# wangxiaohit/GNNPN-SC

Measured on AMD Instinct MI355X. Metric: service-composition problems/sec (ML+2PN inference), higher is better.
Workload: dtype f32-split3xf16 (f32 operands and results; recurrent W_hh.h products: fp32 operands split exactly into 3 x f16, six f16-matrix-core products per term, f32 accumulate; everything else f32 arithmetic)

## Files before the change

gnnpn-sc_amd/csrc/coop_common.h:

```cpp
#pragma once
#include "common.h"
#include "lstm_shared.h"

typedef float f32x4 __attribute__((ext_vector_type(4)));
typedef unsigned long long u64;

__device__ __forceinline__ void granule_store(u64* p, unsigned tag, float v) {
    __hip_atomic_store(p, ((u64)tag << 32) | __float_as_uint(v), __ATOMIC_RELAXED,
                       __HIP_MEMORY_SCOPE_AGENT);
}

typedef unsigned u32x4 __attribute__((ext_vector_type(4)));
#define GNNPN_LD2(dst, voff, sbase, off) "global_load_dwordx4 " dst ", " voff ", " sbase " offset:" off " sc1\n\t"
__device__ __forceinline__ const u64* uniform_ptr(const u64* p) {
    const unsigned long long v = (unsigned long long)p;
    const unsigned lo = __builtin_amdgcn_readfirstlane((unsigned)v), hi = __builtin_amdgcn_readfirstlane((unsigned)(v >> 32));
    return reinterpret_cast<const u64*>(((unsigned long long)hi << 32) | lo);
}
__device__ __forceinline__ void granule_reload2_x8_masked(u32x4 (&v)[8], const u64* base, unsigned voff, unsigned long long lanes) {
    const u64* q = base + 512;
    unsigned long long saved;
    asm volatile("s_and_saveexec_b64 %8, %12\n\t"
                 GNNPN_LD2("%0", "%9", "%10", "0") GNNPN_LD2("%1", "%9", "%10", "1024") GNNPN_LD2("%2", "%9", "%10", "2048")
                 GNNPN_LD2("%3", "%9", "%10", "3072") GNNPN_LD2("%4", "%9", "%11", "0") GNNPN_LD2("%5", "%9", "%11", "1024")
                 GNNPN_LD2("%6", "%9", "%11", "2048") GNNPN_LD2("%7", "%9", "%11", "3072")
                 "s_waitcnt vmcnt(0)\n\t"
                 "s_mov_b64 exec, %8"
                 : "+v"(v[0]), "+v"(v[1]), "+v"(v[2]), "+v"(v[3]), "+v"(v[4]), "+v"(v[5]), "+v"(v[6]), "+v"(v[7]), "=&s"(saved)
                 : "v"(voff), "s"(base), "s"(q), "s"(lanes)
                 : "memory", "scc");
}
__device__ __forceinline__ void granule_load2_x8_x4(u32x4 (&v)[8], u32x4 (&w)[4], const u64* base, const u64* pbase, unsigned voff) {
    const u64* q = base + 512;
    asm volatile(GNNPN_LD2("%0", "%12", "%13", "0") GNNPN_LD2("%1", "%12", "%13", "1024") GNNPN_LD2("%2", "%12", "%13", "2048")
                 GNNPN_LD2("%3", "%12", "%13", "3072") GNNPN_LD2("%4", "%12", "%14", "0") GNNPN_LD2("%5", "%12", "%14", "1024")
                 GNNPN_LD2("%6", "%12", "%14", "2048") GNNPN_LD2("%7", "%12", "%14", "3072")
                 GNNPN_LD2("%8", "%12", "%15", "0") GNNPN_LD2("%9", "%12", "%15", "1024") GNNPN_LD2("%10", "%12", "%15", "2048")
                 GNNPN_LD2("%11", "%12", "%15", "3072")
                 "s_waitcnt vmcnt(0)"
                 : "=&v"(v[0]), "=&v"(v[1]), "=&v"(v[2]), "=&v"(v[3]), "=&v"(v[4]), "=&v"(v[5]), "=&v"(v[6]), "=&v"(v[7]),
                   "=&v"(w[0]), "=&v"(w[1]), "=&v"(w[2]), "=&v"(w[3])
                 : "v"(voff), "s"(base), "s"(q), "s"(pbase)
                 : "memory");
}

__device__ __forceinline__ void granule_load2_x8_x4_lat(u32x4 (&v)[8], u32x4 (&w)[4], u64& lat, const u64* base, const u64* pbase,
                                                        const u64* lbase, unsigned voff) {
    const u64* q = base + 512;
    asm volatile(GNNPN_LD2("%0", "%13", "%15", "0") GNNPN_LD2("%1", "%13", "%15", "1024") GNNPN_LD2("%2", "%13", "%15", "2048")
                 GNNPN_LD2("%3", "%13", "%15", "3072") GNNPN_LD2("%4", "%13", "%16", "0") GNNPN_LD2("%5", "%13", "%16", "1024")
                 GNNPN_LD2("%6", "%13", "%16", "2048") GNNPN_LD2("%7", "%13", "%16", "3072")
                 GNNPN_LD2("%8", "%13", "%17", "0") GNNPN_LD2("%9", "%13", "%17", "1024") GNNPN_LD2("%10", "%13", "%17", "2048")
                 GNNPN_LD2("%11", "%13", "%17", "3072")
                 "global_load_dwordx2 %12, %14, %18 sc1\n\t"
                 "s_waitcnt vmcnt(0)"
                 : "=&v"(v[0]), "=&v"(v[1]), "=&v"(v[2]), "=&v"(v[3]), "=&v"(v[4]), "=&v"(v[5]), "=&v"(v[6]), "=&v"(v[7]),
                   "=&v"(w[0]), "=&v"(w[1]), "=&v"(w[2]), "=&v"(w[3]), "=&v"(lat)
                 : "v"(voff), "v"(voff >> 1), "s"(base), "s"(q), "s"(pbase), "s"(lbase)
                 : "memory");
}

constexpr int COOP_STAFFING_WORD = 8 * 256 + 8;
__device__ __forceinline__ void coop_raise(unsigned* err, unsigned* sticky, unsigned code, unsigned* seats = nullptr) {
    atomicOr(err, code);
    if (sticky) atomicOr(sticky, code);
    if (seats && atomicCAS(err + 4, 1u, 2u) == 1u) atomicSub(seats + COOP_STAFFING_WORD, 1u);
}

constexpr int COOP_STATUS_BYTES = 16384;
constexpr unsigned COOP_LDS_UNITS = 640;
constexpr int COOP_XCD_STRIDE = 32;
constexpr int COOP_XCDCNT_OFFSET = 12288;
constexpr int COOP_ARRIVE_OFFSET = 13312;
constexpr int COOP_PLACED_OFFSET = 14336;
constexpr int COOP_CLAIM_OFFSET = 2048;
constexpr int COOP_TAKEN_OFFSET = 10240;
constexpr int COOP_OVERREAD_BYTES = 4096;
constexpr int COOP_OVERSUB = 3;
constexpr unsigned COOP_SURPLUS_WAIT_TICKS = 1600;
constexpr unsigned COOP_RESERVE_WAIT_TICKS = 200000;

__device__ __forceinline__ unsigned xcc_id() {
// ... 249 lines not shown
        __builtin_amdgcn_sched_barrier(0);
        if (ch == 64 / CH / 2 - 1) mid();
    }
}

typedef _Float16 f16x8 __attribute__((ext_vector_type(8)));
constexpr int LDH16 = 264;
constexpr int SPLIT_TILE = 16 * LDH16;
constexpr float SPLIT_SCALE = 2048.0f, SPLIT_INV = 1.0f / 2048.0f;
constexpr float SPLIT_H_SCALE = 32768.0f, SPLIT_H_INV = 1.0f / 32768.0f;

__device__ __forceinline__ void split3(float xs, _Float16& p0, _Float16& p1, _Float16& p2) {
    p0 = (_Float16)xs;
    const float r1 = __fmul_rn(__fsub_rn(xs, (float)p0), SPLIT_SCALE);
    p1 = (_Float16)r1;
    p2 = (_Float16)__fmul_rn(__fsub_rn(r1, (float)p1), SPLIT_SCALE);
}
__device__ __forceinline__ unsigned short f16_bits(_Float16 v) { return __builtin_bit_cast(unsigned short, v); }

__device__ __forceinline__ unsigned split_tag16(unsigned tag) { return 0x8000u | (tag & 0x7fffu); }
__device__ __forceinline__ u64 split_granule(unsigned tag, float h) {
    _Float16 p0, p1, p2;
    split3(__fmul_rn(h, SPLIT_H_SCALE), p0, p1, p2);
    const unsigned d0 = (unsigned)f16_bits(p0) | (split_tag16(tag) << 16);
    const unsigned d1 = (unsigned)f16_bits(p1) | ((unsigned)f16_bits(p2) << 16);
    return ((u64)d1 << 32) | d0;
}
__device__ __forceinline__ void split_granule_store(u64* p, unsigned tag, float h, bool same_xcd) {
    const u64 g = split_granule(tag, h);
    if (same_xcd) granule_store_l2_bits(p, g);
    else __hip_atomic_store(p, g, __ATOMIC_RELAXED, __HIP_MEMORY_SCOPE_AGENT);
}
__device__ __forceinline__ bool split_pair_tagged(u32x4 v, unsigned tag) {
    const unsigned t = split_tag16(tag);
    return __builtin_amdgcn_perm(v.z, v.x, 0x07060302u) == (t | (t << 16));
}
__device__ __forceinline__ void split_pair_to_lds(_Float16* at, u32x4 v) {
    unsigned* d = reinterpret_cast<unsigned*>(at);
    d[0] = __builtin_amdgcn_perm(v.z, v.x, 0x05040100u);
    d[SPLIT_TILE / 2] = __builtin_amdgcn_perm(v.w, v.y, 0x05040100u);
    d[SPLIT_TILE] = __builtin_amdgcn_perm(v.w, v.y, 0x07060302u);
}
__device__ __forceinline__ void split_store(_Float16* at, float h) {
    _Float16 p0, p1, p2;
    split3(__fmul_rn(h, SPLIT_H_SCALE), p0, p1, p2);
    at[0] = p0;
    at[SPLIT_TILE] = p1;
    at[2 * SPLIT_TILE] = p2;
}

constexpr int SPLIT_WT_DWORDS = 4 * 8 * 64 * 4;
template <int HD>
__device__ __forceinline__ float split_weights(const float* __restrict__ Wp, int gate, int u, int kq, f16x8 (&w0)[8],
                                               f16x8 (&w1)[8], unsigned* wt) {
    float m = 0.0f;
#pragma unroll
    for (int kk = 0; kk < 8; ++kk)
#pragma unroll
        for (int j = 0; j < 8; ++j)
            m = fmaxf(m, fabsf(Wp[((size_t)((8 * kk + 2 * kq + (j >> 2)) * 4 + gate) * HD + u) * 4 + (j & 3)]));
    m = fmaxf(m, __shfl_xor(m, 16, 64));
    m = fmaxf(m, __shfl_xor(m, 32, 64));
    int e = 0;
    if (m > 0.0f && m < 3.0e38f) (void)frexpf(m, &e);
    int s = m > 0.0f ? 15 - e : 0;
    s = s > 96 ? 96 : (s < -96 ? -96 : s);
    const float up = ldexpf(1.0f, s);
#pragma unroll
    for (int kk = 0; kk < 8; ++kk) {
        unsigned bytes[2] = {0u, 0u};
#pragma unroll
        for (int j = 0; j < 8; ++j) {
            const float w = Wp[((size_t)((8 * kk + 2 * kq + (j >> 2)) * 4 + gate) * HD + u) * 4 + (j & 3)];
            _Float16 p0, p1, p2;
            split3(__fmul_rn(w, up), p0, p1, p2);
            w0[kk][j] = p0;
            w1[kk][j] = p1;
            bytes[j >> 2] |= (unsigned)(f16_bits(p2) >> 8) << (8 * (j & 3));
        }
        wt[4 * 64 * kk] = bytes[0];
        wt[4 * 64 * kk + 1] = bytes[1];
    }
    return ldexpf(1.0f, -(15 + s));
}
constexpr int SPLIT_PACK_U4_PER_MEMBER = 2 * 2 * 8 * 256 + 8 * 256 + 2 * 256 / 4;
constexpr int SPLIT_PACK_MEMBERS = 8;
__device__ __forceinline__ void load_split_weights(const uint4* __restrict__ pk, int tid, f16x8 (&w0)[2][8], f16x8 (&w1)[2][8],
                                                   unsigned* wt_lane, float (&inv)[2]) {
#pragma unroll
    for (int tl = 0; tl < 2; ++tl)
#pragma unroll
        for (int kk = 0; kk < 8; ++kk) {
            w0[tl][kk] = __builtin_bit_cast(f16x8, pk[((tl * 2 + 0) * 8 + kk) * 256 + tid]);
            w1[tl][kk] = __builtin_bit_cast(f16x8, pk[((tl * 2 + 1) * 8 + kk) * 256 + tid]);
        }
#pragma unroll
    for (int kk = 0; kk < 8; ++kk) *reinterpret_cast<uint4*>(wt_lane + 4 * 64 * kk) = pk[8192 + kk * 256 + tid];
    const float* fi = reinterpret_cast<const float*>(pk + 10240);
    inv[0] = fi[tid];
    inv[1] = fi[256 + tid];
}

__device__ __forceinline__ f16x8 split_expand(unsigned lo, unsigned hi) {
    const u32x4 r = {__builtin_amdgcn_perm(0u, lo, 0x010c000cu), __builtin_amdgcn_perm(0u, lo, 0x030c020cu),
                     __builtin_amdgcn_perm(0u, hi, 0x010c000cu), __builtin_amdgcn_perm(0u, hi, 0x030c020cu)};
    return __builtin_bit_cast(f16x8, r);
}
template <typename Mid = NoHook>
__device__ __forceinline__ void split_chain(const _Float16* base, const f16x8 (&w0)[2][8], const f16x8 (&w1)[2][8],
                                            const unsigned* wt, const float (&inv)[2], f32x4 (&acc)[2], Mid mid = Mid()) {
    constexpr int NT = 2;
    f32x4 a0[NT], a0b[NT], a1[NT], a2[NT];
#pragma unroll
    for (int n = 0; n < NT; ++n) a0[n] = a0b[n] = a1[n] = a2[n] = f32x4{0.f, 0.f, 0.f, 0.f};
    f16x8 h0[2];
    h0[0] = *reinterpret_cast<const f16x8*>(base);
    f16x8 h1 = *reinterpret_cast<const f16x8*>(base + SPLIT_TILE);
    f16x8 h2 = *reinterpret_cast<const f16x8*>(base + 2 * SPLIT_TILE);
    u32x4 t = *reinterpret_cast<const u32x4*>(wt);
#define GNNPN_FENCE __builtin_amdgcn_sched_barrier(0)
#pragma unroll
    for (int kk = 0; kk < 8; ++kk) {
        const int nx = 32 * (kk + 1), cur = kk & 1;
        u32x4 e0, e1;
        if (kk < 7) h0[cur ^ 1] = *reinterpret_cast<const f16x8*>(base + nx);
        GNNPN_FENCE;
        a2[0] = __builtin_amdgcn_mfma_f32_16x16x32_f16(h1, w1[0][kk], a2[0], 0, 0, 0);
        e0.x = __builtin_amdgcn_perm(0u, t.x, 0x010c000cu);
        e0.y = __builtin_amdgcn_perm(0u, t.x, 0x030c020cu);
        GNNPN_FENCE;
        a2[1] = __builtin_amdgcn_mfma_f32_16x16x32_f16(h1, w1[1][kk], a2[1], 0, 0, 0);
        e0.z = __builtin_amdgcn_perm(0u, t.y, 0x010c000cu);
        e0.w = __builtin_amdgcn_perm(0u, t.y, 0x030c020cu);
        GNNPN_FENCE;
        a1[0] = __builtin_amdgcn_mfma_f32_16x16x32_f16(h1, w0[0][kk], a1[0], 0, 0, 0);
        e1.x = __builtin_amdgcn_perm(0u, t.z, 0x010c000cu);
        e1.y = __builtin_amdgcn_perm(0u, t.z, 0x030c020cu);
        GNNPN_FENCE;
        a1[1] = __builtin_amdgcn_mfma_f32_16x16x32_f16(h1, w0[1][kk], a1[1], 0, 0, 0);
        e1.z = __builtin_amdgcn_perm(0u, t.w, 0x010c000cu);
        e1.w = __builtin_amdgcn_perm(0u, t.w, 0x030c020cu);
        GNNPN_FENCE;
        if (kk < 7) {
            h1 = *reinterpret_cast<const f16x8*>(base + SPLIT_TILE + nx);
            t = *reinterpret_cast<const u32x4*>(wt + 4 * 64 * (kk + 1));
        }
        a2[0] = __builtin_amdgcn_mfma_f32_16x16x32_f16(h0[cur], __builtin_bit_cast(f16x8, e0), a2[0], 0, 0, 0);
        GNNPN_FENCE;
        a2[1] = __builtin_amdgcn_mfma_f32_16x16x32_f16(h0[cur], __builtin_bit_cast(f16x8, e1), a2[1], 0, 0, 0);
        GNNPN_FENCE;
        if (kk < 4) a0[0] = __builtin_amdgcn_mfma_f32_16x16x32_f16(h0[cur], w0[0][kk], a0[0], 0, 0, 0);
        else a0b[0] = __builtin_amdgcn_mfma_f32_16x16x32_f16(h0[cur], w0[0][kk], a0b[0], 0, 0, 0);
        GNNPN_FENCE;
        if (kk < 4) a0[1] = __builtin_amdgcn_mfma_f32_16x16x32_f16(h0[cur], w0[1][kk], a0[1], 0, 0, 0);
        else a0b[1] = __builtin_amdgcn_mfma_f32_16x16x32_f16(h0[cur], w0[1][kk], a0b[1], 0, 0, 0);
        GNNPN_FENCE;
        a2[0] = __builtin_amdgcn_mfma_f32_16x16x32_f16(h2, w0[0][kk], a2[0], 0, 0, 0);
        GNNPN_FENCE;
        a2[1] = __builtin_amdgcn_mfma_f32_16x16x32_f16(h2, w0[1][kk], a2[1], 0, 0, 0);
        GNNPN_FENCE;
        if (kk < 7) h2 = *reinterpret_cast<const f16x8*>(base + 2 * SPLIT_TILE + nx);
        a1[0] = __builtin_amdgcn_mfma_f32_16x16x32_f16(h0[cur], w1[0][kk], a1[0], 0, 0, 0);
        GNNPN_FENCE;
        a1[1] = __builtin_amdgcn_mfma_f32_16x16x32_f16(h0[cur], w1[1][kk], a1[1], 0, 0, 0);
        GNNPN_FENCE;
        if (kk == 3) mid();
    }
#undef GNNPN_FENCE
#pragma unroll
    for (int n = 0; n < NT; ++n)
#pragma unroll
        for (int r = 0; r < 4; ++r)
            acc[n][r] = __fmul_rn(fmaf(fmaf(a2[n][r], SPLIT_INV, a1[n][r]), SPLIT_INV, __fadd_rn(a0[n][r], a0b[n][r])), inv[n]);
}

__device__ __forceinline__ void cell_update_split(const f32x2 (&g0)[2], const f32x2 (&g1)[2], bool lo_half, f32x2& cst, f32x2& h) {
    f32x2 a0[2], a1[2];
#pragma unroll
    for (int q = 0; q < 2; ++q) {
        a0[q] = cell_act2(g0[q], false);
        a1[q] = cell_act2(g1[q], lo_half);
    }
    const f32x2 s0 = lo_half ? a0[1] : a0[0], s1 = lo_half ? a1[1] : a1[0];
    const f32x2 t0 = {swap8(s0.x), swap8(s0.y)}, t1 = {swap8(s1.x), swap8(s1.y)};
    const f32x2 ig = lo_half ? a0[0] : t0, gg = lo_half ? a1[0] : t1;
    const f32x2 fg = lo_half ? t0 : a0[1], og = lo_half ? t1 : a1[1];
    cst = fg * cst + ig * gg;
    h = og * cell_act2(cst, true);
}
```

gnnpn-sc_amd/csrc/lstm_coop.hip:

```cpp
#include "common.h"
#include "recurrent.h"
#include "lstm_shared.h"
#include "coop_common.h"
#include "decode_shared.h"

namespace {
constexpr int H = COOP_H;
constexpr int G = COOP_G;
constexpr int ROWS = COOP_ROWS;
constexpr int UNITS = H / G;
constexpr unsigned SPIN_LIMIT = 400000;
constexpr int GROUP_GRANULES = 2 * ROWS * H + 2 * 4 * G;
constexpr int ENC_LOOP_PAD_NOPS = 13;
}

template <int PREC>
__device__ __forceinline__ bool sweep_quarter(const u64* buf, unsigned tag, float* hs, int wave, int lane, bool keep,
                                              bool nowait = false) {
    const u64* src = uniform_ptr(buf + wave * 4 * H);
    const unsigned voff = 16u * lane;
    u32x4 v[8];
#pragma unroll
    for (int j = 0; j < 8; ++j) asm volatile("" : "=v"(v[j]));
    bool bad = true;
    unsigned spins = 0;
    int nap = 1;
    for (;;) {
        granule_reload2_x8_masked(v, src, voff, __ballot(bad));
        bad = false;
#pragma unroll
        for (int j = 0; j < 8; ++j) {
            if constexpr (PREC == 2) bad |= !split_pair_tagged(v[j], tag);
            else bad |= (v[j].y != tag) | (v[j].w != tag);
        }
        if (!__any(bad) || nowait) break;
        if (++spins > SPIN_LIMIT) return false;
        for (int z = 0; z < nap; ++z) __builtin_amdgcn_s_sleep(2);
        if (nap < 16) nap <<= 1;
    }
    if (keep) {
#pragma unroll
        for (int j = 0; j < 8; ++j) {
            const int i = 2 * (j * 64 + lane);
            if constexpr (PREC == 0) {
                float* d = &hs[ht_index(wave * 4 + (i >> 8), i & 255)];
                d[0] = __uint_as_float(v[j].x);
                d[64] = __uint_as_float(v[j].z);
            } else {
                _Float16* h16 = reinterpret_cast<_Float16*>(hs) + (wave * 4 + (i >> 8)) * LDH16 + (i & 255);
                if constexpr (PREC == 2) {
                    split_pair_to_lds(h16, v[j]);
                } else {
                    h16[0] = (_Float16)__uint_as_float(v[j].x);
                    h16[1] = (_Float16)__uint_as_float(v[j].z);
                }
            }
        }
    }
    return true;
}


template <int PREC, bool PRE, bool DIAG>
__global__ __launch_bounds__(256, 2) void lstm_encode_coop_kernel(LstmNets nets, u64* __restrict__ xchg,
                                                                  unsigned* __restrict__ err, unsigned* __restrict__ sticky,
                                                                  int32_t B, int32_t L, int n_nets, int groups_per_net,
                                                                  int gpx, int ablate_arg, unsigned* __restrict__ seats,
                                                                  unsigned* __restrict__ diag) {
    const int ablate = DIAG ? (ablate_arg & ~0x1000) : (ablate_arg & 128);
    constexpr bool F16 = PREC != 0, SPLIT = PREC == 2;
    constexpr int HS_FLOATS = PREC == 2 ? 3 * SPLIT_TILE / 2 : ROWS * LDH16;
    __shared__ __attribute__((aligned(16))) float hs[HS_FLOATS];
    __shared__ __attribute__((aligned(16))) float hst[ROWS][UNITS];
    __shared__ int abort_flag;

    const int lane = threadIdx.x & 63, wave = threadIdx.x >> 6;
    const int kq = lane >> 4, c = lane & 15;
    __shared__ int place[2];
    int group, member;
    u64 p_entry = 0, p_placed = 0, p_weights = 0;
    if constexpr (DIAG) p_entry = phase_stamp();
    if (!coop_place<G>(err, gpx, place, group, member, seats, (ablate_arg & 0x1000) != 0, sticky)) return;
    if constexpr (DIAG) p_placed = phase_stamp();
    const int net = group / groups_per_net, gi = group % groups_per_net;
    if (net >= n_nets) return;
    if (threadIdx.x == 0) abort_flag = 0;
    __syncthreads();
    const bool same_xcd = !(ablate & 128);
    if (threadIdx.x == 0 && same_xcd) atomicAdd(err + COOP_PLACED_OFFSET / 4 + COOP_XCD_STRIDE * xcc_id(), 1u);

    const float* __restrict__ pre = PRE ? nets.pregates[net] : nullptr;
    const float* __restrict__ xin = nets.inputs[net];
    const float* __restrict__ Wp = nets.whh[net];
    float* __restrict__ enc = nets.enc_out[net];
    u64* xg = xchg + (size_t)group * GROUP_GRANULES;

    const int unit = member * UNITS + wave * 8 + (c & 7);
    int wrow[2];
    wrow[0] = (0 + (c >> 3)) * H + unit;
    wrow[1] = (2 + (c >> 3)) * H + unit;
    float wB[F16 ? 1 : 2][F16 ? 1 : 64], bh[2], wX[2][2] = {{0.f, 0.f}, {0.f, 0.f}}, bx[2] = {0.f, 0.f};
    f16x8 wB16[F16 ? 2 : 1][8];
    f16x8 wL16[SPLIT ? 2 : 1][8];
    float winv[2] = {1.0f, 1.0f};
    __shared__ __attribute__((aligned(16))) unsigned wts[SPLIT ? SPLIT_WT_DWORDS : 4];
    unsigned* wt_lane = wts + (SPLIT ? (wave * 8 * 64 + lane) * 4 : 0);
    const uint4* __restrict__ Wsplit = SPLIT ? static_cast<const uint4*>(nets.whh_split[net]) : nullptr;
    if constexpr (SPLIT) {
        if (Wsplit) load_split_weights(Wsplit + (size_t)member * SPLIT_PACK_U4_PER_MEMBER, threadIdx.x, wB16, wL16, wt_lane, winv);
    }
#pragma unroll
    for (int tl = 0; tl < 2; ++tl) {
        const int gate = wrow[tl] / H, u = wrow[tl] % H;
        bh[tl] = nets.bhh[net][wrow[tl]];
        if constexpr (SPLIT) {
            if (!Wsplit) winv[tl] = split_weights<H>(Wp, gate, u, kq, wB16[tl], wL16[tl], wt_lane + 2 * tl);
        } else if constexpr (F16) {
#pragma unroll
            for (int kk = 0; kk < 8; ++kk)
#pragma unroll
                for (int j = 0; j < 8; ++j)
                    wB16[tl][kk][j] = (_Float16)Wp[((size_t)((8 * kk + 2 * kq + (j >> 2)) * 4 + gate) * H + u) * 4 + (j & 3)];
        }
        if constexpr (!PRE) {
            wX[tl][0] = nets.w_in[net][wrow[tl] * 8 + kq];
            wX[tl][1] = nets.w_in[net][wrow[tl] * 8 + 4 + kq];
            bx[tl] = nets.b_in[net][wrow[tl]];
        }
        if constexpr (!F16) {
#pragma unroll
            for (int kk = 0; kk < 64; ++kk)
                wB[tl][kk] = Wp[((size_t)(kk * 4 + gate) * H + u) * 4 + kq];
        }
    }

    if constexpr (DIAG) {
        asm volatile("" ::"v"(winv[0]), "v"(winv[1]), "v"(bh[0]), "v"(bh[1]));
        p_weights = phase_stamp();
    }
    const int n_tiles = (B + ROWS - 1) / ROWS;
    unsigned step = 0;
    unsigned tiles_done = 0;
    bool first_tile = true;
    for (int tile = gi; tile < n_tiles; tile += groups_per_net) {
        const int b0 = tile * ROWS;
        f32x2 cst = {0.f, 0.f};
        f32x2 hlast = {0.f, 0.f};
        float pg[2][4], pg_next[2][4] = {{0.f, 0.f, 0.f, 0.f}, {0.f, 0.f, 0.f, 0.f}};
        float ax[2] = {0.f, 0.f}, ax_next[2] = {0.f, 0.f};
        auto load_input = [&](int t, float (&pgv)[2][4], float (&axv)[2]) {
            if constexpr (PRE) {
#pragma unroll
                for (int r = 0; r < 4; ++r) {
                    const int b = b0 + kq * 4 + r;
#pragma unroll
                    for (int tl = 0; tl < 2; ++tl)
                        pgv[tl][r] = b < B ? pre[((int64_t)b * L + t) * (4 * H) + wrow[tl]] : 0.0f;
                }
            } else if (b0 + c < B) {
                const float* row = xin + ((int64_t)(b0 + c) * L + t) * 8;
                axv[0] = row[kq];
                axv[1] = row[4 + kq];
            }
        };
        load_input(0, pg_next, ax_next);
#ifndef GNNPN_ENC_PAD_NOPS
#define GNNPN_ENC_PAD_NOPS ENC_LOOP_PAD_NOPS
#endif
        if constexpr (SPLIT && !DIAG) asm volatile(".p2align 6\n\t.rept %0\n\ts_nop 0\n\t.endr" ::"n"(GNNPN_ENC_PAD_NOPS) : "memory");
        for (int t = 0; t < L; ++t, ++step) {
            const bool stamps = ablate & 32;
            u64 s0 = 0, s1 = 0, s2 = 0, s3 = 0, s4 = 0, s5 = 0;
            if (stamps) s0 = phase_stamp();
#pragma unroll
            for (int tl = 0; tl < 2; ++tl) {
                ax[tl] = ax_next[tl];
#pragma unroll
                for (int r = 0; r < 4; ++r) pg[tl][r] = pg_next[tl][r];
            }
            f32x4 px0 = {0.f, 0.f, 0.f, 0.f}, px1 = {0.f, 0.f, 0.f, 0.f};
            if constexpr (!PRE) {
                px0 = __builtin_amdgcn_mfma_f32_16x16x4f32(ax[0], wX[0][0], px0, 0, 0, 0);
                px1 = __builtin_amdgcn_mfma_f32_16x16x4f32(ax[0], wX[1][0], px1, 0, 0, 0);
                px0 = __builtin_amdgcn_mfma_f32_16x16x4f32(ax[1], wX[0][1], px0, 0, 0, 0);
                px1 = __builtin_amdgcn_mfma_f32_16x16x4f32(ax[1], wX[1][1], px1, 0, 0, 0);
            }
            bool ok = true;
            if (t == 0) {
                for (int i = threadIdx.x; i < HS_FLOATS; i += 256) hs[i] = 0.0f;
                if (!first_tile) ok = sweep_quarter<PREC>(xg + ((step - 1) & 1) * (ROWS * H), step, hs, wave, lane, false);
            } else if (!(ablate & 8)) {
                ok = sweep_quarter<PREC>(xg + ((step - 1) & 1) * (ROWS * H), step, hs, wave, lane, true, ablate & 4);
            }
            if (!ok) abort_flag = 1;
            if constexpr (DIAG) {
                if (!ok && lane == 0 && diag) {
                    const unsigned n = atomicAdd(diag, 1u);
                    if (n < 31) {
                        unsigned* rec = diag + 16 * (n + 1);
                        const unsigned* cnt = err + COOP_XCDCNT_OFFSET / 4;
                        const unsigned* arr = err + COOP_ARRIVE_OFFSET / 4;
                        unsigned c0 = 0, c1 = 0, a0 = 0, a1 = 0;
                        for (int x = 0; x < 4; ++x) {
                            c0 |= (cnt[COOP_XCD_STRIDE * x] & 0xffu) << (8 * x);
                            c1 |= (cnt[COOP_XCD_STRIDE * (4 + x)] & 0xffu) << (8 * x);
                            a0 |= (arr[COOP_XCD_STRIDE * x] & 0xffu) << (8 * x);
                            a1 |= (arr[COOP_XCD_STRIDE * (4 + x)] & 0xffu) << (8 * x);
                        }
                        rec[0] = group; rec[1] = member; rec[2] = tile; rec[3] = t; rec[4] = wave; rec[5] = step;
                        rec[6] = 0; rec[7] = 0xE0Cu; rec[8] = 0; rec[9] = c0; rec[10] = c1; rec[11] = a0; rec[12] = a1;
                        rec[13] = gpx; rec[14] = blockIdx.x; rec[15] = err[0];
                    }
                }
            }
            if (stamps) s1 = phase_stamp();
            __syncthreads();
            if (abort_flag) break;
            if (stamps) s2 = phase_stamp();
            f32x4 acc0 = {0.f, 0.f, 0.f, 0.f}, acc1 = {0.f, 0.f, 0.f, 0.f};
            u64 s2a = 0;
            if (stamps) s2a = phase_stamp();
            if constexpr (SPLIT) {
                if (t > 0) {
                    f32x4 acc[2] = {acc0, acc1};
                    split_chain(reinterpret_cast<const _Float16*>(hs) + c * LDH16 + 8 * kq, wB16, wL16, wt_lane, winv, acc);
                    acc0 = acc[0];
                    acc1 = acc[1];
                }
            } else if constexpr (F16) {
                if (t > 0) {
                    const _Float16* base = reinterpret_cast<const _Float16*>(hs) + c * LDH16 + 8 * kq;
                    f16x8 a16[8];
#pragma unroll
                    for (int kk = 0; kk < 8; ++kk) a16[kk] = *reinterpret_cast<const f16x8*>(base + 32 * kk);
#pragma unroll
                    for (int kk = 0; kk < 8; ++kk) {
                        acc0 = __builtin_amdgcn_mfma_f32_16x16x32_f16(a16[kk], wB16[0][kk], acc0, 0, 0, 0);
                        acc1 = __builtin_amdgcn_mfma_f32_16x16x32_f16(a16[kk], wB16[1][kk], acc1, 0, 0, 0);
                    }
                }
            } else {
                if (t > 0 && !(ablate & 1)) mfma_chain_pair<LDT, 16, true>(hs, c, kq, wB[0], wB[F16 ? 0 : 1], acc0, acc1);
            }
            if (t + 1 < L && !(ablate & 0x400)) load_input(t + 1, pg_next, ax_next);
            if (t > 0 && threadIdx.x < ROWS * 8 && !(ablate & 0x200)) {
                const int row = threadIdx.x >> 3, q = threadIdx.x & 7;
                if (b0 + row < B)
                    *reinterpret_cast<float4*>(enc + ((int64_t)(b0 + row) * L + (t - 1)) * H + member * UNITS + 4 * q) =
                        *reinterpret_cast<const float4*>(&hst[row][4 * q]);
            }

            if (stamps) {
                asm volatile("" ::"v"(acc0[0]), "v"(acc1[0]));
                s3 = phase_stamp();
            }
            if constexpr (!PRE) {
#pragma unroll
                for (int r = 0; r < 4; ++r) {
                    pg[0][r] = __fadd_rn(px0[r], bx[0]);
                    pg[1][r] = __fadd_rn(px1[r], bx[1]);
                }
            }
            __syncthreads();
            if (stamps) s4 = phase_stamp();

            u64* out_buf = xg + (step & 1) * (ROWS * H);
            {
                f32x2 g0[2], g1[2];
#pragma unroll
                for (int q = 0; q < 2; ++q) {
                    g0[q] = (f32x2{acc0[2 * q], acc0[2 * q + 1]} + pk_set(bh[0])) + f32x2{pg[0][2 * q], pg[0][2 * q + 1]};
                    g1[q] = (f32x2{acc1[2 * q], acc1[2 * q + 1]} + pk_set(bh[1])) + f32x2{pg[1][2 * q], pg[1][2 * q + 1]};
                }
                cell_update_split(g0, g1, c < 8, cst, hlast);
            }
            {
                const int r0 = kq * 4 + (c < 8 ? 0 : 2);
                u64* dst = out_buf + r0 * H + unit;
                if constexpr (SPLIT) {
                    split_granule_store(dst, step + 1, hlast.x, same_xcd);
                    split_granule_store(dst + H, step + 1, hlast.y, same_xcd);
                } else if (!(ablate & 16)) {
                    if (same_xcd) {
                        granule_store_l2(dst, step + 1, hlast.x);
                        granule_store_l2(dst + H, step + 1, hlast.y);
                    } else {
                        granule_store(dst, step + 1, hlast.x);
                        granule_store(dst + H, step + 1, hlast.y);
                    }
                }
                hst[r0][wave * 8 + (c & 7)] = hlast.x;
                hst[r0 + 1][wave * 8 + (c & 7)] = hlast.y;
            }
            if (stamps) {
                asm volatile("" ::"v"(hlast.y));
                s5 = phase_stamp();
                if (blockIdx.x == 0 && threadIdx.x == 0 && t > 0) {
                    u64* prof = reinterpret_cast<u64*>(err) + 4;
                    prof[0] += s1 - s0;
                    prof[1] += s2 - s1;
                    prof[2] += s3 - s2;
                    prof[6] += s2a - s2;
                    prof[3] += s4 - s3;
                    prof[4] += s5 - s4;
                    prof[5] += 1;
                    if (t == 1 && first_tile) {
                        prof[7] = p_placed - p_entry;
                        prof[8] = p_weights - p_placed;
                        prof[9] = s0 - p_weights;
                    }
                }
            }
        }
        if (abort_flag) break;
        __syncthreads();
        if (threadIdx.x < ROWS * 8) {
            const int row = threadIdx.x >> 3, q = threadIdx.x & 7;
            if (b0 + row < B)
                *reinterpret_cast<float4*>(enc + ((int64_t)(b0 + row) * L + (L - 1)) * H + member * UNITS + 4 * q) =
                    *reinterpret_cast<const float4*>(&hst[row][4 * q]);
        }
#pragma unroll
        for (int r = 0; r < 2; ++r) {
            const int b = b0 + kq * 4 + (c < 8 ? 0 : 2) + r;
            if (b < B) {
                nets.h_n[net][(int64_t)b * H + unit] = r ? hlast.y : hlast.x;
                nets.c_n[net][(int64_t)b * H + unit] = r ? cst.y : cst.x;
            }
        }
        first_tile = false;
        ++tiles_done;
    }
    if (threadIdx.x == 0) {
        if (abort_flag) coop_raise(err, sticky, 1u, seats);
        coop_note_finished(sticky, GNNPN_STATUS_ENC_FINISHED, tiles_done);
    }
}


__global__ __launch_bounds__(256) void lstm_pack_split_kernel(const float* __restrict__ Wp, uint4* __restrict__ out) {
    __shared__ __attribute__((aligned(16))) unsigned wts[SPLIT_WT_DWORDS];
    const int tid = threadIdx.x, lane = tid & 63, wave = tid >> 6, kq = lane >> 4, c = lane & 15;
    const int member = blockIdx.x;
    const int unit = member * UNITS + wave * 8 + (c & 7);
    f16x8 w0[2][8], w1[2][8];
    float inv[2];
    unsigned* wt_lane = wts + (wave * 8 * 64 + lane) * 4;
#pragma unroll
    for (int tl = 0; tl < 2; ++tl) inv[tl] = split_weights<H>(Wp, 2 * tl + (c >> 3), unit, kq, w0[tl], w1[tl], wt_lane + 2 * tl);
    uint4* pk = out + (size_t)member * SPLIT_PACK_U4_PER_MEMBER;
#pragma unroll
    for (int tl = 0; tl < 2; ++tl)
#pragma unroll
        for (int kk = 0; kk < 8; ++kk) {
            pk[((tl * 2 + 0) * 8 + kk) * 256 + tid] = __builtin_bit_cast(uint4, w0[tl][kk]);
            pk[((tl * 2 + 1) * 8 + kk) * 256 + tid] = __builtin_bit_cast(uint4, w1[tl][kk]);
        }
#pragma unroll
    for (int kk = 0; kk < 8; ++kk) pk[8192 + kk * 256 + tid] = *reinterpret_cast<const uint4*>(wt_lane + 4 * 64 * kk);
    float* fi = reinterpret_cast<float*>(pk + 10240);
    fi[tid] = inv[0];
    fi[256 + tid] = inv[1];
}

extern "C" int64_t gnnpn_lstm_split_weights_bytes(void) { return (int64_t)SPLIT_PACK_MEMBERS * SPLIT_PACK_U4_PER_MEMBER * 16; }

extern "C" int gnnpn_lstm_pack_split_weights_f32(const float* whh_packed, void* split, void* stream) {
    GNNPN_REQUIRE(whh_packed && split, "lstm_pack_split_weights: null operand");
    GNNPN_REQUIRE(gnnpn_aligned(whh_packed, 16) && gnnpn_aligned(split, 16), "lstm_pack_split_weights: operands must be 16-byte aligned");
    static_assert(G == SPLIT_PACK_MEMBERS, "one packed block per group member");
    hipLaunchKernelGGL(lstm_pack_split_kernel, dim3(G), dim3(256), 0, (hipStream_t)stream, whh_packed, static_cast<uint4*>(split));
    GNNPN_CHECK_LAUNCH("lstm_pack_split_weights");
    return GNNPN_OK;
}

static int64_t encode_workspace_bytes(int groups) { return COOP_STATUS_BYTES + (int64_t)groups * GROUP_GRANULES * sizeof(u64); }

extern "C" int64_t gnnpn_lstm_encode_workspace_bytes(void) {
    (void)gnnpn_cu_seat_table();
    return encode_workspace_bytes(64);
}

int gnnpn_launch_encode_coop(const LstmNets& nets, int n_nets, int32_t B, int32_t L, int precision, const CoopOpts& opts,
                             void* workspace, int64_t workspace_bytes, hipStream_t s) {
    bool pre = nets.pregates[0] != nullptr;
    for (int n = 0; n < n_nets; ++n)
        if ((nets.pregates[n] != nullptr) != pre)
            GNNPN_FAIL(GNNPN_E_ARG, "lstm_encode: all nets of a call must use the same input-side form");
    const int prec = precision;
    const int abl = (gnnpn_option_lstm_ablate() & ~(0x800 | 0x1000 | 0x2000)) | (opts.write_through ? 128 : 0);
    const bool diag = (abl & ~128) != 0;
    if (diag && (prec == 1 || pre || (prec == 2 && (abl & ~(128 | 32)) != 0)))
        GNNPN_FAIL(GNNPN_E_UNSUP, "lstm_encode: diagnostics are built for the folded form (fp32: all switches; split: stamps only)");
    CoopLaunch c;
    if (const int rc = coop_begin("lstm_encode", n_nets, B, encode_workspace_bytes, GNNPN_STATUS_ENC_EXPECTED, opts, workspace,
                                  workspace_bytes, s, c))
        return rc;
    u64* p_x = reinterpret_cast<u64*>(c.buffers);
    const int abl_arg = abl | (opts.paired_start ? 0x1000 : 0);
    static unsigned* p_diag = gnnpn_decode_diag_buffer();
#define GNNPN_ENC(PREC_, PRE_, DIAG_)                                                                                        \
    hipLaunchKernelGGL((lstm_encode_coop_kernel<PREC_, PRE_, DIAG_>), dim3(COOP_OVERSUB * c.groups * G), dim3(256),             \
                       gnnpn_lds_padding((const void*)lstm_encode_coop_kernel<PREC_, PRE_, DIAG_>, opts.lds_kb), s, nets, p_x, \
                       c.status, opts.sticky, B, L, n_nets, c.groups_per_net, c.gpx, abl_arg, c.seats, p_diag)
    if (diag) {
        if (prec == 2) GNNPN_ENC(2, false, true);
        else GNNPN_ENC(0, false, true);
    } else if (prec == 2 && pre) GNNPN_ENC(2, true, false);
    else if (prec == 2) GNNPN_ENC(2, false, false);
    else if (prec == 1 && pre) GNNPN_ENC(1, true, false);
    else if (prec == 1) GNNPN_ENC(1, false, false);
    else if (pre) GNNPN_ENC(0, true, false);
    else GNNPN_ENC(0, false, false);
#undef GNNPN_ENC
    return GNNPN_OK;
}
```

Before: 479,300.

## Split LSTM encoder recurrence across eight waves with one gate tile each

Measured after the change: 383,500. 20.0% lower.

```diff
diff --git a/gnnpn-sc_amd/csrc/coop_common.h b/gnnpn-sc_amd/csrc/coop_common.h
--- a/gnnpn-sc_amd/csrc/coop_common.h
+++ b/gnnpn-sc_amd/csrc/coop_common.h
@@ -12,10 +12,11 @@
 
 typedef unsigned u32x4 __attribute__((ext_vector_type(4)));
 #define GNNPN_LD2(dst, voff, sbase, off) "global_load_dwordx4 " dst ", " voff ", " sbase " offset:" off " sc1\n\t"
-__device__ __forceinline__ const u64* uniform_ptr(const u64* p) {
+template <typename T>
+__device__ __forceinline__ T* uniform_ptr(T* p) {
     const unsigned long long v = (unsigned long long)p;
     const unsigned lo = __builtin_amdgcn_readfirstlane((unsigned)v), hi = __builtin_amdgcn_readfirstlane((unsigned)(v >> 32));
-    return reinterpret_cast<const u64*>(((unsigned long long)hi << 32) | lo);
+    return reinterpret_cast<T*>(((unsigned long long)hi << 32) | lo);
 }
 __device__ __forceinline__ void granule_reload2_x8_masked(u32x4 (&v)[8], const u64* base, unsigned voff, unsigned long long lanes) {
     const u64* q = base + 512;
@@ -28,6 +29,17 @@
                  "s_mov_b64 exec, %8"
                  : "+v"(v[0]), "+v"(v[1]), "+v"(v[2]), "+v"(v[3]), "+v"(v[4]), "+v"(v[5]), "+v"(v[6]), "+v"(v[7]), "=&s"(saved)
                  : "v"(voff), "s"(base), "s"(q), "s"(lanes)
+                 : "memory", "scc");
+}
+__device__ __forceinline__ void granule_reload2_x4_masked(u32x4 (&v)[4], const u64* base, unsigned voff, unsigned long long lanes) {
+    unsigned long long saved;
+    asm volatile("s_and_saveexec_b64 %4, %7\n\t"
+                 GNNPN_LD2("%0", "%5", "%6", "0") GNNPN_LD2("%1", "%5", "%6", "1024") GNNPN_LD2("%2", "%5", "%6", "2048")
+                 GNNPN_LD2("%3", "%5", "%6", "3072")
+                 "s_waitcnt vmcnt(0)\n\t"
+                 "s_mov_b64 exec, %4"
+                 : "+v"(v[0]), "+v"(v[1]), "+v"(v[2]), "+v"(v[3]), "=&s"(saved)
+                 : "v"(voff), "s"(base), "s"(lanes)
                  : "memory", "scc");
 }
 __device__ __forceinline__ void granule_load2_x8_x4(u32x4 (&v)[8], u32x4 (&w)[4], const u64* base, const u64* pbase, unsigned voff) {
@@ -383,7 +395,7 @@
 constexpr int SPLIT_WT_DWORDS = 4 * 8 * 64 * 4;
 template <int HD>
 __device__ __forceinline__ float split_weights(const float* __restrict__ Wp, int gate, int u, int kq, f16x8 (&w0)[8],
-                                               f16x8 (&w1)[8], unsigned* wt) {
+                                               f16x8 (&w1)[8], unsigned* wt, int wt_stride = 4 * 64) {
     float m = 0.0f;
 #pragma unroll
     for (int kk = 0; kk < 8; ++kk)
@@ -409,8 +421,8 @@
             w1[kk][j] = p1;
             bytes[j >> 2] |= (unsigned)(f16_bits(p2) >> 8) << (8 * (j & 3));
         }
-        wt[4 * 64 * kk] = bytes[0];
-        wt[4 * 64 * kk + 1] = bytes[1];
+        wt[wt_stride * kk] = bytes[0];
+        wt[wt_stride * kk + 1] = bytes[1];
     }
     return ldexpf(1.0f, -(15 + s));
 }
@@ -430,6 +442,20 @@
     const float* fi = reinterpret_cast<const float*>(pk + 10240);
     inv[0] = fi[tid];
     inv[1] = fi[256 + tid];
+}
+
+__device__ __forceinline__ float load_split_weights_tile(const uint4* __restrict__ pk, int gate, int u, int kq, f16x8 (&w0)[8],
+                                                         f16x8 (&w1)[8], unsigned* wt_lane) {
+    const int tl = gate >> 1, tid = 64 * ((u & 31) >> 3) + 16 * kq + (((gate & 1) << 3) | (u & 7));
+#pragma unroll
+    for (int kk = 0; kk < 8; ++kk) {
+        w0[kk] = __builtin_bit_cast(f16x8, pk[((tl * 2 + 0) * 8 + kk) * 256 + tid]);
+        w1[kk] = __builtin_bit_cast(f16x8, pk[((tl * 2 + 1) * 8 + kk) * 256 + tid]);
+    }
+#pragma unroll
+    for (int kk = 0; kk < 8; ++kk)
+        *reinterpret_cast<uint2*>(wt_lane + 2 * 64 * kk) = reinterpret_cast<const uint2*>(pk + 8192 + kk * 256 + tid)[tl];
+    return reinterpret_cast<const float*>(pk + 10240)[tl * 256 + tid];
 }
 
 __device__ __forceinline__ f16x8 split_expand(unsigned lo, unsigned hi) {
@@ -503,6 +529,48 @@
 #pragma unroll
         for (int r = 0; r < 4; ++r)
             acc[n][r] = __fmul_rn(fmaf(fmaf(a2[n][r], SPLIT_INV, a1[n][r]), SPLIT_INV, __fadd_rn(a0[n][r], a0b[n][r])), inv[n]);
+}
+
+__device__ __forceinline__ void split_chain_tile(const _Float16* base, const f16x8 (&w0)[8], const f16x8 (&w1)[8], const unsigned* wt,
+                                                 f32x4& acc) {
+    f32x4 a0 = {0.f, 0.f, 0.f, 0.f}, a0b = a0, a1 = a0, a2 = a0;
+    f16x8 h0 = *reinterpret_cast<const f16x8*>(base);
+    f16x8 h1 = *reinterpret_cast<const f16x8*>(base + SPLIT_TILE);
+    f16x8 h2 = *reinterpret_cast<const f16x8*>(base + 2 * SPLIT_TILE);
+    uint2 t = *reinterpret_cast<const uint2*>(wt);
+#define GNNPN_FENCE __builtin_amdgcn_sched_barrier(0)
+#pragma unroll
+    for (int kk = 0; kk < 8; ++kk) {
+        const int nx = 32 * (kk + 1);
+        u32x4 e;
+        GNNPN_FENCE;
+        a2 = __builtin_amdgcn_mfma_f32_16x16x32_f16(h1, w1[kk], a2, 0, 0, 0);
+        e.x = __builtin_amdgcn_perm(0u, t.x, 0x010c000cu);
+        e.y = __builtin_amdgcn_perm(0u, t.x, 0x030c020cu);
+        GNNPN_FENCE;
+        a1 = __builtin_amdgcn_mfma_f32_16x16x32_f16(h1, w0[kk], a1, 0, 0, 0);
+        e.z = __builtin_amdgcn_perm(0u, t.y, 0x010c000cu);
+        e.w = __builtin_amdgcn_perm(0u, t.y, 0x030c020cu);
+        GNNPN_FENCE;
+        if (kk < 7) {
+            h1 = *reinterpret_cast<const f16x8*>(base + SPLIT_TILE + nx);
+            t = *reinterpret_cast<const uint2*>(wt + 2 * 64 * (kk + 1));
+        }
+        a2 = __builtin_amdgcn_mfma_f32_16x16x32_f16(h0, __builtin_bit_cast(f16x8, e), a2, 0, 0, 0);
+        GNNPN_FENCE;
+        if (kk < 4) a0 = __builtin_amdgcn_mfma_f32_16x16x32_f16(h0, w0[kk], a0, 0, 0, 0);
+        else a0b = __builtin_amdgcn_mfma_f32_16x16x32_f16(h0, w0[kk], a0b, 0, 0, 0);
+        GNNPN_FENCE;
+        a2 = __builtin_amdgcn_mfma_f32_16x16x32_f16(h2, w0[kk], a2, 0, 0, 0);
+        GNNPN_FENCE;
+        if (kk < 7) h2 = *reinterpret_cast<const f16x8*>(base + 2 * SPLIT_TILE + nx);
+        a1 = __builtin_amdgcn_mfma_f32_16x16x32_f16(h0, w1[kk], a1, 0, 0, 0);
+        GNNPN_FENCE;
+        if (kk < 7) h0 = *reinterpret_cast<const f16x8*>(base + nx);
+    }
+#undef GNNPN_FENCE
+#pragma unroll
+    for (int r = 0; r < 4; ++r) acc[r] = fmaf(fmaf(a2[r], SPLIT_INV, a1[r]), SPLIT_INV, __fadd_rn(a0[r], a0b[r]));
 }
 
 __device__ __forceinline__ void cell_update_split(const f32x2 (&g0)[2], const f32x2 (&g1)[2], bool lo_half, f32x2& cst, f32x2& h) {
@@ -519,3 +587,29 @@
     cst = fg * cst + ig * gg;
     h = og * cell_act2(cst, true);
 }
+
+template <int D>
+__device__ __forceinline__ float quad_from(float v) {
+    constexpr int ctrl = ((0 + D) & 3) | (((1 + D) & 3) << 2) | (((2 + D) & 3) << 4) | (((3 + D) & 3) << 6);
+    return __int_as_float(__builtin_amdgcn_update_dpp(0, __float_as_int(v), ctrl, 0xF, 0xF, false));
+}
+__device__ __forceinline__ void cell_update_quad(const f32x2 (&g)[2], int q, float& cst, float& h) {
+    const f32x2 a01 = cell_act2(g[0], q == 2), a23 = cell_act2(g[1], q == 2);
+    const float a[4] = {a01.x, a01.y, a23.x, a23.y};
+    const bool b0 = q & 1, b1 = q & 2;
+    float r[4], s[4], t[4], u[4], gate[4];
+#pragma unroll
+    for (int j = 0; j < 4; ++j) r[j] = b0 ? a[(j + 1) & 3] : a[j];
+#pragma unroll
+    for (int j = 0; j < 4; ++j) s[j] = b1 ? r[(j + 2) & 3] : r[j];
+    t[0] = s[0];
+    t[1] = quad_from<1>(s[3]);
+    t[2] = quad_from<2>(s[2]);
+    t[3] = quad_from<3>(s[1]);
+#pragma unroll
+    for (int j = 0; j < 4; ++j) u[j] = b0 ? t[(j + 3) & 3] : t[j];
+#pragma unroll
+    for (int j = 0; j < 4; ++j) gate[j] = b1 ? u[(j + 2) & 3] : u[j];
+    cst = __fadd_rn(__fmul_rn(gate[1], cst), __fmul_rn(gate[0], gate[2]));
+    h = __fmul_rn(gate[3], cell_act(cst, true));
+}
diff --git a/gnnpn-sc_amd/csrc/lstm_coop.hip b/gnnpn-sc_amd/csrc/lstm_coop.hip
--- a/gnnpn-sc_amd/csrc/lstm_coop.hip
+++ b/gnnpn-sc_amd/csrc/lstm_coop.hip
@@ -12,6 +12,7 @@
 constexpr unsigned SPIN_LIMIT = 400000;
 constexpr int GROUP_GRANULES = 2 * ROWS * H + 2 * 4 * G;
 constexpr int ENC_LOOP_PAD_NOPS = 13;
+constexpr int enc_waves(int prec) { return prec == 2 ? 8 : 4; }
 }
 
 template <int PREC>
@@ -60,9 +61,37 @@
     return true;
 }
 
+__device__ __forceinline__ bool sweep_row_pair(const u64* buf, unsigned tag, float* hs, int wave, int lane, bool keep) {
+    const u64* src = uniform_ptr(buf + wave * 2 * H);
+    const unsigned voff = 16u * lane;
+    u32x4 v[4];
+#pragma unroll
+    for (int j = 0; j < 4; ++j) asm volatile("" : "=v"(v[j]));
+    bool bad = true;
+    unsigned spins = 0;
+    int nap = 1;
+    for (;;) {
+        granule_reload2_x4_masked(v, src, voff, __ballot(bad));
+        bad = false;
+#pragma unroll
+        for (int j = 0; j < 4; ++j) bad |= !split_pair_tagged(v[j], tag);
+        if (!__any(bad)) break;
+        if (++spins > SPIN_LIMIT) return false;
+        for (int z = 0; z < nap; ++z) __builtin_amdgcn_s_sleep(2);
+        if (nap < 16) nap <<= 1;
+    }
+    if (keep) {
+#pragma unroll
+        for (int j = 0; j < 4; ++j) {
+            const int i = 2 * (j * 64 + lane);
+            split_pair_to_lds(reinterpret_cast<_Float16*>(hs) + (wave * 2 + (i >> 8)) * LDH16 + (i & 255), v[j]);
+        }
+    }
+    return true;
+}
 
 template <int PREC, bool PRE, bool DIAG>
-__global__ __launch_bounds__(256, 2) void lstm_encode_coop_kernel(LstmNets nets, u64* __restrict__ xchg,
+__global__ __launch_bounds__(64 * enc_waves(PREC), enc_waves(PREC) / 2) void lstm_encode_coop_kernel(LstmNets nets, u64* __restrict__ xchg,
                                                                   unsigned* __restrict__ err, unsigned* __restrict__ sticky,
                                                                   int32_t B, int32_t L, int n_nets, int groups_per_net,
                                                                   int gpx, int ablate_arg, unsigned* __restrict__ seats,
@@ -82,6 +111,10 @@
     if constexpr (DIAG) p_entry = phase_stamp();
     if (!coop_place<G>(err, gpx, place, group, member, seats, (ablate_arg & 0x1000) != 0, sticky)) return;
     if constexpr (DIAG) p_placed = phase_stamp();
+    if constexpr (SPLIT) {
+        group = __builtin_amdgcn_readfirstlane(group);
+        member = __builtin_amdgcn_readfirstlane(member);
+    }
     const int net = group / groups_per_net, gi = group % groups_per_net;
     if (net >= n_nets) return;
     if (threadIdx.x == 0) abort_flag = 0;
@@ -93,28 +126,35 @@
     const float* __restrict__ xin = nets.inputs[net];
     const float* __restrict__ Wp = nets.whh[net];
     float* __restrict__ enc = nets.enc_out[net];
+    float* __restrict__ out_h = nets.h_n[net];
+    float* __restrict__ out_c = nets.c_n[net];
     u64* xg = xchg + (size_t)group * GROUP_GRANULES;
 
-    const int unit = member * UNITS + wave * 8 + (c & 7);
-    int wrow[2];
-    wrow[0] = (0 + (c >> 3)) * H + unit;
-    wrow[1] = (2 + (c >> 3)) * H + unit;
-    float wB[F16 ? 1 : 2][F16 ? 1 : 64], bh[2], wX[2][2] = {{0.f, 0.f}, {0.f, 0.f}}, bx[2] = {0.f, 0.f};
-    f16x8 wB16[F16 ? 2 : 1][8];
-    f16x8 wL16[SPLIT ? 2 : 1][8];
-    float winv[2] = {1.0f, 1.0f};
+    constexpr int TILES = SPLIT ? 1 : 2, WAVES = enc_waves(PREC);
+    const int unit = SPLIT ? member * UNITS + wave * 4 + (c >> 2) : member * UNITS + wave * 8 + (c & 7);
+    int wrow[TILES];
+    if constexpr (SPLIT) {
+        wrow[0] = (c & 3) * H + unit;
+    } else {
+        wrow[0] = (0 + (c >> 3)) * H + unit;
+        wrow[TILES - 1] = (2 + (c >> 3)) * H + unit;
+    }
+    float wB[F16 ? 1 : 2][F16 ? 1 : 64], bh[TILES], wX[TILES][2], bx[TILES];
+    f16x8 wB16[F16 && !SPLIT ? 2 : 1][8];
+    f16x8 wS0[8], wS1[8];
+    float winv = 1.0f;
     __shared__ __attribute__((aligned(16))) unsigned wts[SPLIT ? SPLIT_WT_DWORDS : 4];
-    unsigned* wt_lane = wts + (SPLIT ? (wave * 8 * 64 + lane) * 4 : 0);
+    static_assert(!SPLIT || SPLIT_WT_DWORDS == WAVES * 8 * 64 * 2, "byte image: [wave][k-block][lane]{lo, hi}");
+    unsigned* wt_lane = wts + (SPLIT ? wave * 8 * 64 * 2 + lane * 2 : 0);
     const uint4* __restrict__ Wsplit = SPLIT ? static_cast<const uint4*>(nets.whh_split[net]) : nullptr;
-    if constexpr (SPLIT) {
-        if (Wsplit) load_split_weights(Wsplit + (size_t)member * SPLIT_PACK_U4_PER_MEMBER, threadIdx.x, wB16, wL16, wt_lane, winv);
-    }
-#pragma unroll
-    for (int tl = 0; tl < 2; ++tl) {
+#pragma unroll
+    for (int tl = 0; tl < TILES; ++tl) {
         const int gate = wrow[tl] / H, u = wrow[tl] % H;
         bh[tl] = nets.bhh[net][wrow[tl]];
+        wX[tl][0] = wX[tl][1] = bx[tl] = 0.f;
         if constexpr (SPLIT) {
-            if (!Wsplit) winv[tl] = split_weights<H>(Wp, gate, u, kq, wB16[tl], wL16[tl], wt_lane + 2 * tl);
+            if (Wsplit) winv = load_split_weights_tile(Wsplit + (size_t)member * SPLIT_PACK_U4_PER_MEMBER, gate, u, kq, wS0, wS1, wt_lane);
+            else winv = split_weights<H>(Wp, gate, u, kq, wS0, wS1, wt_lane, 2 * 64);
         } else if constexpr (F16) {
 #pragma unroll
             for (int kk = 0; kk < 8; ++kk)
@@ -135,7 +175,7 @@
     }
 
     if constexpr (DIAG) {
-        asm volatile("" ::"v"(winv[0]), "v"(winv[1]), "v"(bh[0]), "v"(bh[1]));
+        asm volatile("" ::"v"(winv), "v"(bh[0]), "v"(bh[TILES - 1]));
         p_weights = phase_stamp();
     }
     const int n_tiles = (B + ROWS - 1) / ROWS;
@@ -146,16 +186,21 @@
         const int b0 = tile * ROWS;
         f32x2 cst = {0.f, 0.f};
         f32x2 hlast = {0.f, 0.f};
-        float pg[2][4], pg_next[2][4] = {{0.f, 0.f, 0.f, 0.f}, {0.f, 0.f, 0.f, 0.f}};
+        float cs1 = 0.f, h1 = 0.f;
+        float pg[TILES][4], pg_next[TILES][4];
+#pragma unroll
+        for (int tl = 0; tl < TILES; ++tl)
+#pragma unroll
+            for (int r = 0; r < 4; ++r) pg_next[tl][r] = 0.f;
         float ax[2] = {0.f, 0.f}, ax_next[2] = {0.f, 0.f};
-        auto load_input = [&](int t, float (&pgv)[2][4], float (&axv)[2]) {
+        auto load_input = [&](int t, float (&pgv)[TILES][4], float (&axv)[2], int kq, int c, int wr0) {
             if constexpr (PRE) {
 #pragma unroll
                 for (int r = 0; r < 4; ++r) {
                     const int b = b0 + kq * 4 + r;
 #pragma unroll
-                    for (int tl = 0; tl < 2; ++tl)
-                        pgv[tl][r] = b < B ? pre[((int64_t)b * L + t) * (4 * H) + wrow[tl]] : 0.0f;
+                    for (int tl = 0; tl < TILES; ++tl)
+                        pgv[tl][r] = b < B ? pre[((int64_t)b * L + t) * (4 * H) + (SPLIT ? wr0 : wrow[tl])] : 0.0f;
                 }
             } else if (b0 + c < B) {
                 const float* row = xin + ((int64_t)(b0 + c) * L + t) * 8;
@@ -163,32 +208,43 @@
                 axv[1] = row[4 + kq];
             }
         };
-        load_input(0, pg_next, ax_next);
+        load_input(0, pg_next, ax_next, kq, c, wrow[0]);
 #ifndef GNNPN_ENC_PAD_NOPS
 #define GNNPN_ENC_PAD_NOPS ENC_LOOP_PAD_NOPS
 #endif
         if constexpr (SPLIT && !DIAG) asm volatile(".p2align 6\n\t.rept %0\n\ts_nop 0\n\t.endr" ::"n"(GNNPN_ENC_PAD_NOPS) : "memory");
         for (int t = 0; t < L; ++t, ++step) {
+            int tid_v = threadIdx.x;
+            if constexpr (SPLIT) asm volatile("" : "+v"(tid_v));
+            const int lane = tid_v & 63, wave = SPLIT ? __builtin_amdgcn_readfirstlane(tid_v >> 6) : tid_v >> 6;
+            const int kq = lane >> 4, c = lane & 15;
+            const int unit = SPLIT ? member * UNITS + wave * 4 + (c >> 2) : member * UNITS + wave * 8 + (c & 7);
             const bool stamps = ablate & 32;
             u64 s0 = 0, s1 = 0, s2 = 0, s3 = 0, s4 = 0, s5 = 0;
             if (stamps) s0 = phase_stamp();
-#pragma unroll
-            for (int tl = 0; tl < 2; ++tl) {
-                ax[tl] = ax_next[tl];
+            ax[0] = ax_next[0];
+            ax[1] = ax_next[1];
+#pragma unroll
+            for (int tl = 0; tl < TILES; ++tl)
 #pragma unroll
                 for (int r = 0; r < 4; ++r) pg[tl][r] = pg_next[tl][r];
-            }
             f32x4 px0 = {0.f, 0.f, 0.f, 0.f}, px1 = {0.f, 0.f, 0.f, 0.f};
             if constexpr (!PRE) {
                 px0 = __builtin_amdgcn_mfma_f32_16x16x4f32(ax[0], wX[0][0], px0, 0, 0, 0);
-                px1 = __builtin_amdgcn_mfma_f32_16x16x4f32(ax[0], wX[1][0], px1, 0, 0, 0);
+                if constexpr (!SPLIT) px1 = __builtin_amdgcn_mfma_f32_16x16x4f32(ax[0], wX[TILES - 1][0], px1, 0, 0, 0);
                 px0 = __builtin_amdgcn_mfma_f32_16x16x4f32(ax[1], wX[0][1], px0, 0, 0, 0);
-                px1 = __builtin_amdgcn_mfma_f32_16x16x4f32(ax[1], wX[1][1], px1, 0, 0, 0);
+                if constexpr (!SPLIT) px1 = __builtin_amdgcn_mfma_f32_16x16x4f32(ax[1], wX[TILES - 1][1], px1, 0, 0, 0);
             }
             bool ok = true;
             if (t == 0) {
-                for (int i = threadIdx.x; i < HS_FLOATS; i += 256) hs[i] = 0.0f;
-                if (!first_tile) ok = sweep_quarter<PREC>(xg + ((step - 1) & 1) * (ROWS * H), step, hs, wave, lane, false);
+                for (int i = tid_v; i < HS_FLOATS; i += 64 * WAVES) hs[i] = 0.0f;
+                if constexpr (SPLIT) {
+                    if (!first_tile) ok = sweep_row_pair(xg + ((step - 1) & 1) * (ROWS * H), step, hs, wave, lane, false);
+                } else {
+                    if (!first_tile) ok = sweep_quarter<PREC>(xg + ((step - 1) & 1) * (ROWS * H), step, hs, wave, lane, false);
+                }
+            } else if constexpr (SPLIT) {
+                ok = sweep_row_pair(xg + ((step - 1) & 1) * (ROWS * H), step, hs, wave, lane, true);
             } else if (!(ablate & 8)) {
                 ok = sweep_quarter<PREC>(xg + ((step - 1) & 1) * (ROWS * H), step, hs, wave, lane, true, ablate & 4);
             }
@@ -221,12 +277,7 @@
             u64 s2a = 0;
             if (stamps) s2a = phase_stamp();
             if constexpr (SPLIT) {
-                if (t > 0) {
-                    f32x4 acc[2] = {acc0, acc1};
-                    split_chain(reinterpret_cast<const _Float16*>(hs) + c * LDH16 + 8 * kq, wB16, wL16, wt_lane, winv, acc);
-                    acc0 = acc[0];
-                    acc1 = acc[1];
-                }
+                if (t > 0) split_chain_tile(reinterpret_cast<const _Float16*>(hs) + c * LDH16 + 8 * kq, wS0, wS1, wt_lane, acc0);
             } else if constexpr (F16) {
                 if (t > 0) {
                     const _Float16* base = reinterpret_cast<const _Float16*>(hs) + c * LDH16 + 8 * kq;
@@ -242,9 +293,15 @@
             } else {
                 if (t > 0 && !(ablate & 1)) mfma_chain_pair<LDT, 16, true>(hs, c, kq, wB[0], wB[F16 ? 0 : 1], acc0, acc1);
             }
-            if (t + 1 < L && !(ablate & 0x400)) load_input(t + 1, pg_next, ax_next);
-            if (t > 0 && threadIdx.x < ROWS * 8 && !(ablate & 0x200)) {
-                const int row = threadIdx.x >> 3, q = threadIdx.x & 7;
+            int tid_w = tid_v;
+            if constexpr (SPLIT) asm volatile("" : "+v"(tid_w));
+            {
+            const int lane = tid_w & 63, wave = SPLIT ? __builtin_amdgcn_readfirstlane(tid_w >> 6) : tid_w >> 6;
+            const int kq = lane >> 4, c = lane & 15;
+            const int unit = SPLIT ? member * UNITS + wave * 4 + (c >> 2) : member * UNITS + wave * 8 + (c & 7);
+            if (t + 1 < L && !(ablate & 0x400)) load_input(t + 1, pg_next, ax_next, kq, c, (c & 3) * H + unit);
+            if (t > 0 && tid_w < ROWS * 8 && !(ablate & 0x200)) {
+                const int row = tid_w >> 3, q = tid_w & 7;
                 if (b0 + row < B)
                     *reinterpret_cast<float4*>(enc + ((int64_t)(b0 + row) * L + (t - 1)) * H + member * UNITS + 4 * q) =
                         *reinterpret_cast<const float4*>(&hst[row][4 * q]);
@@ -255,32 +312,44 @@
                 s3 = phase_stamp();
             }
             if constexpr (!PRE) {
+                float bx1 = bx[0];
+                if constexpr (SPLIT) asm volatile("" : "+v"(bx1));
 #pragma unroll
                 for (int r = 0; r < 4; ++r) {
-                    pg[0][r] = __fadd_rn(px0[r], bx[0]);
-                    pg[1][r] = __fadd_rn(px1[r], bx[1]);
+                    pg[0][r] = __fadd_rn(px0[r], bx1);
+                    if constexpr (!SPLIT) pg[TILES - 1][r] = __fadd_rn(px1[r], bx[TILES - 1]);
                 }
             }
             __syncthreads();
             if (stamps) s4 = phase_stamp();
 
             u64* out_buf = xg + (step & 1) * (ROWS * H);
-            {
+            if constexpr (SPLIT) {
+                f32x2 g0[2];
+                float inv1 = winv, bh1 = bh[0];
+                asm volatile("" : "+v"(inv1), "+v"(bh1));
+#pragma unroll
+                for (int r = 0; r < 4; ++r) acc0[r] = __fmul_rn(acc0[r], inv1);
+#pragma unroll
+                for (int q = 0; q < 2; ++q)
+                    g0[q] = (f32x2{acc0[2 * q], acc0[2 * q + 1]} + pk_set(bh1)) + f32x2{pg[0][2 * q], pg[0][2 * q + 1]};
+                int q = c & 3;
+                asm volatile("" : "+v"(q));
+                cell_update_quad(g0, q, cs1, h1);
+                const int r0 = kq * 4 + (c & 3);
+                split_granule_store(out_buf + r0 * H + unit, step + 1, h1, same_xcd);
+                hst[r0][wave * 4 + (c >> 2)] = h1;
+            } else {
                 f32x2 g0[2], g1[2];
 #pragma unroll
                 for (int q = 0; q < 2; ++q) {
                     g0[q] = (f32x2{acc0[2 * q], acc0[2 * q + 1]} + pk_set(bh[0])) + f32x2{pg[0][2 * q], pg[0][2 * q + 1]};
-                    g1[q] = (f32x2{acc1[2 * q], acc1[2 * q + 1]} + pk_set(bh[1])) + f32x2{pg[1][2 * q], pg[1][2 * q + 1]};
+                    g1[q] = (f32x2{acc1[2 * q], acc1[2 * q + 1]} + pk_set(bh[TILES - 1])) + f32x2{pg[TILES - 1][2 * q], pg[TILES - 1][2 * q + 1]};
                 }
                 cell_update_split(g0, g1, c < 8, cst, hlast);
-            }
-            {
                 const int r0 = kq * 4 + (c < 8 ? 0 : 2);
                 u64* dst = out_buf + r0 * H + unit;
-                if constexpr (SPLIT) {
-                    split_granule_store(dst, step + 1, hlast.x, same_xcd);
-                    split_granule_store(dst + H, step + 1, hlast.y, same_xcd);
-                } else if (!(ablate & 16)) {
+                if (!(ablate & 16)) {
                     if (same_xcd) {
                         granule_store_l2(dst, step + 1, hlast.x);
                         granule_store_l2(dst + H, step + 1, hlast.y);
@@ -293,7 +362,7 @@
                 hst[r0 + 1][wave * 8 + (c & 7)] = hlast.y;
             }
             if (stamps) {
-                asm volatile("" ::"v"(hlast.y));
+                asm volatile("" ::"v"(hlast.y), "v"(h1));
                 s5 = phase_stamp();
                 if (blockIdx.x == 0 && threadIdx.x == 0 && t > 0) {
                     u64* prof = reinterpret_cast<u64*>(err) + 4;
@@ -311,6 +380,7 @@
                     }
                 }
             }
+            }
         }
         if (abort_flag) break;
         __syncthreads();
@@ -320,12 +390,20 @@
                 *reinterpret_cast<float4*>(enc + ((int64_t)(b0 + row) * L + (L - 1)) * H + member * UNITS + 4 * q) =
                     *reinterpret_cast<const float4*>(&hst[row][4 * q]);
         }
-#pragma unroll
-        for (int r = 0; r < 2; ++r) {
-            const int b = b0 + kq * 4 + (c < 8 ? 0 : 2) + r;
+        if constexpr (SPLIT) {
+            const int b = b0 + kq * 4 + (c & 3);
             if (b < B) {
-                nets.h_n[net][(int64_t)b * H + unit] = r ? hlast.y : hlast.x;
-                nets.c_n[net][(int64_t)b * H + unit] = r ? cst.y : cst.x;
+                out_h[(int64_t)b * H + unit] = h1;
+                out_c[(int64_t)b * H + unit] = cs1;
+            }
+        } else {
+#pragma unroll
+            for (int r = 0; r < 2; ++r) {
+                const int b = b0 + kq * 4 + (c < 8 ? 0 : 2) + r;
+                if (b < B) {
+                    out_h[(int64_t)b * H + unit] = r ? hlast.y : hlast.x;
+                    out_c[(int64_t)b * H + unit] = r ? cst.y : cst.x;
+                }
             }
         }
         first_tile = false;
@@ -400,7 +478,7 @@
     const int abl_arg = abl | (opts.paired_start ? 0x1000 : 0);
     static unsigned* p_diag = gnnpn_decode_diag_buffer();
 #define GNNPN_ENC(PREC_, PRE_, DIAG_)                                                                                        \
-    hipLaunchKernelGGL((lstm_encode_coop_kernel<PREC_, PRE_, DIAG_>), dim3(COOP_OVERSUB * c.groups * G), dim3(256),             \
+    hipLaunchKernelGGL((lstm_encode_coop_kernel<PREC_, PRE_, DIAG_>), dim3(COOP_OVERSUB * c.groups * G), dim3(64 * enc_waves(PREC_)), \
                        gnnpn_lds_padding((const void*)lstm_encode_coop_kernel<PREC_, PRE_, DIAG_>, opts.lds_kb), s, nets, p_x, \
                        c.status, opts.sticky, B, L, n_nets, c.groups_per_net, c.gpx, abl_arg, c.seats, p_diag)
     if (diag) {
```
